# invesalius/invesalius3

Measured on AMD Instinct MI355X. Metric: Mvoxel/s segmentation + Mtriangles/s marching-cubes, 512^3 int16, 1/2/4/8 GPU, higher is better.
Workload: dtype i16; 1 GPU; configs[1]: 512x512x512 int16 per GPU, threshold(226..3071) + 26-neighbour region-grow + marching-cubes(mask@127); global_voxels=134217728, parallelism=z-slab x1, collectives=none, overlap=none

## Files before the change

### invesalius3_amd/csrc/k_flood.hip

```cpp
#include <math.h>
#include <map>
#include <mutex>
#include <stdlib.h>

#include "flood_tiles.h"

typedef short short8_t __attribute__((ext_vector_type(8)));

namespace {

constexpr int NT = TY * TZ;
constexpr int HY = TY + 2, HZ = TZ + 2;
constexpr int BATCH = 8;
constexpr int SUB = 1;
constexpr unsigned int CLOSED = 0x40u;

template <typename T> __device__ __forceinline__ double as_double(T v) { return (double)v; }

template <typename T, int BAR>
__global__ __launch_bounds__(256) void k_flood_candidates16(const short8_t *__restrict__ data,
                                                            const uint4 *__restrict__ bar, int64_t nchunks, double t0,
                                                            double t1, double fill, uint16_t *__restrict__ cand) {
    const int64_t stride = (int64_t)gridDim.x * blockDim.x;
    const int lo = (int)ceil(t0 < -70000.0 ? -70000.0 : t0), hi = (int)floor(t1 > 70000.0 ? 70000.0 : t1);
    const unsigned fb = (unsigned)(uint8_t)fill;
    for (int64_t c = (int64_t)blockIdx.x * blockDim.x + threadIdx.x; c < nchunks; c += stride) {
        const short8_t a = __builtin_nontemporal_load(&data[2 * c]);
        const short8_t b = __builtin_nontemporal_load(&data[2 * c + 1]);
        uint4 q = make_uint4(0, 0, 0, 0);
        if (BAR == 1) q = bar[c];
        const unsigned bw[4] = {q.x, q.y, q.z, q.w};
        unsigned m = 0;
#pragma unroll
        for (int e = 0; e < 16; e++) {
            const int v = (int)(T)(e < 8 ? a[e & 7] : b[e & 7]);
            bool ok = v >= lo && v <= hi;
            if (BAR == 1) ok = ok && ((bw[e >> 2] >> (8 * (e & 3))) & 0xffu) != fb;
            if (BAR == 2) ok = ok && (double)v != fill;
            m |= ok ? (1u << e) : 0u;
        }
        cand[c] = (uint16_t)m;
    }
}

template <int BAR>
__global__ __launch_bounds__(256) void k_flood_candidates16_ranges(const short8_t *__restrict__ data,
                                                                   const uint4 *__restrict__ bar,
                                                                   const unsigned *__restrict__ ranges, int64_t nchunks,
                                                                   double t0, double t1, double fill,
                                                                   uint16_t *__restrict__ cand) {
    const int64_t stride = (int64_t)gridDim.x * blockDim.x;
    const int lo = (int)ceil(t0 < -70000.0 ? -70000.0 : t0), hi = (int)floor(t1 > 70000.0 ? 70000.0 : t1);
    const unsigned fb = (unsigned)(uint8_t)fill;
    int64_t c = (int64_t)blockIdx.x * blockDim.x + threadIdx.x;
    if (c >= nchunks) return;
    unsigned rec = ranges[c >> 2];
    for (;;) {
        const int64_t cn = c + stride;
        unsigned rec_next = 0;
        if (cn < nchunks) rec_next = ranges[cn >> 2];
        const int mn = (int)(short)(rec & 0xffffu), mx = (int)(short)(rec >> 16);
        unsigned m = 0;
        if (!(mx < lo || mn > hi)) {
            const bool inside = mn >= lo && mx <= hi;
            if (inside) {
                m = 0xffffu;
            } else {
                const short8_t a = __builtin_nontemporal_load(&data[2 * c]);
                const short8_t b = __builtin_nontemporal_load(&data[2 * c + 1]);
#pragma unroll
                for (int e = 0; e < 16; e++) {
                    const int v = (int)(e < 8 ? a[e & 7] : b[e & 7]);
                    m |= (v >= lo && v <= hi) ? (1u << e) : 0u;
                }
            }
            if (BAR == 1 && m) {
                const uint4 q = bar[c];
                const unsigned bw[4] = {q.x, q.y, q.z, q.w};
#pragma unroll
                for (int e = 0; e < 16; e++)
                    if (((bw[e >> 2] >> (8 * (e & 3))) & 0xffu) == fb) m &= ~(1u << e);
            }
        }
        cand[c] = (uint16_t)m;
        if (cn >= nchunks) break;
        c = cn;
        rec = rec_next;
    }
}

template <typename T, int BAR>
__global__ __launch_bounds__(256) void k_flood_candidates(const T *__restrict__ data, const uint8_t *__restrict__ bar,
                                                          Tiles t, double t0, double t1, double fill,
                                                          uint8_t *__restrict__ cand) {
    const int64_t bpr = t.wx * 8;
    const int64_t total = t.dz * t.dy * bpr;
    const int64_t stride = (int64_t)gridDim.x * blockDim.x;
    const bool vec = (sizeof(T) == 2) && (t.dx % 8 == 0) && (((uintptr_t)data & 15) == 0) &&
                     (BAR != 1 || ((uintptr_t)bar & 7) == 0);
    for (int64_t i = (int64_t)blockIdx.x * blockDim.x + threadIdx.x; i < total; i += stride) {
        const int64_t row = i / bpr, q = i - row * bpr;
        const int64_t x0 = q * 8;
        unsigned m = 0;
        if (x0 < t.dx) {
            const int64_t base = row * t.dx + x0;
            if (vec) {
                const short8_t v = *reinterpret_cast<const short8_t *>(data + base);
                unsigned long long b8 = 0;
                if (BAR == 1) b8 = *reinterpret_cast<const unsigned long long *>(bar + base);
#pragma unroll
                for (int e = 0; e < 8; e++) {
                    const double d = (double)(T)v[e];
                    bool ok = d >= t0 && d <= t1;
                    if (BAR == 1) ok = ok && (((b8 >> (8 * e)) & 0xff) != (unsigned long long)(uint8_t)fill);
                    if (BAR == 2) ok = ok && d != fill;
                    m |= ok ? (1u << e) : 0u;
                }
            } else {
#pragma unroll
                for (int e = 0; e < 8; e++) {
                    if (x0 + e < t.dx) {
                        const double d = as_double(data[base + e]);
                        bool ok = d >= t0 && d <= t1;
                        if (BAR == 1) ok = ok && bar[base + e] != (uint8_t)fill;
                        if (BAR == 2) ok = ok && d != fill;
                        m |= ok ? (1u << e) : 0u;
                    }
                }
            }
        }
        cand[i] = (uint8_t)m;
    }
}

template <typename T>
__global__ void k_flood_seed(const T *__restrict__ data, Tiles t, double t0, double t1, const int64_t *__restrict__ seeds,
                             int64_t nseeds, unsigned long long *__restrict__ cand,
                             unsigned long long *__restrict__ reached, uint8_t *__restrict__ dirty) {
    const int64_t n = (int64_t)blockIdx.x * blockDim.x + threadIdx.x;
    if (n >= nseeds) return;
    const int64_t x = seeds[3 * n], y = seeds[3 * n + 1], z = seeds[3 * n + 2];
    const double v = as_double(data[(z * t.dy + y) * t.dx + x]);
    if (!(v >= t0 && v <= t1)) return;
    const int64_t w = (z * t.dy + y) * t.wx + (x >> 6);
    const unsigned long long bit = 1ull << (x & 63);
    atomicOr(&cand[w], bit);
    atomicOr(&reached[w], bit);
    mark_tile_nbhd(t, dirty, z / TZ, y / TY, x >> 6);
}

struct SeedPack {
    int64_t xyz[16][3];
    int n;
};
template <typename T>
__global__ void k_flood_seed_args(const T *__restrict__ data, Tiles t, double t0, double t1, SeedPack sp,
                                  unsigned long long *__restrict__ cand, unsigned long long *__restrict__ reached,
                                  uint8_t *__restrict__ dirty) {
    const int n = threadIdx.x;
    if (n >= sp.n) return;
    const int64_t x = sp.xyz[n][0], y = sp.xyz[n][1], z = sp.xyz[n][2];
    const double v = as_double(data[(z * t.dy + y) * t.dx + x]);
    if (!(v >= t0 && v <= t1)) return;
    const int64_t w = (z * t.dy + y) * t.wx + (x >> 6);
    const unsigned long long bit = 1ull << (x & 63);
    atomicOr(&cand[w], bit);
    atomicOr(&reached[w], bit);
    mark_tile_nbhd(t, dirty, z / TZ, y / TY, x >> 6);
}

__device__ __forceinline__ unsigned long long fill_up(unsigned long long seed, unsigned long long m) {
    return (((m + seed) ^ m) & m) | seed;
}
__device__ __forceinline__ unsigned long long fill_runs(unsigned long long seed, unsigned long long m) {
    unsigned long long f = fill_up(seed, m);
    return __brevll(fill_up(__brevll(f), __brevll(m)));
}

__device__ __forceinline__ void lds_barrier() {
    __builtin_amdgcn_s_waitcnt(0xC07F);
    __builtin_amdgcn_s_barrier();
}
struct TileOpen {
    unsigned long long sO[HZ * HY];
};
struct TileLds {
    unsigned long long sN[HZ * HY];
    unsigned long long sD[HZ * HY];
    unsigned char sCL[HZ * HY], sCR[HZ * HY];
    unsigned int dirs;
    unsigned int open;
    unsigned int vote[2];
};
__device__ __forceinline__ void post_dirs(TileLds &L, unsigned dirs) {
#pragma unroll
    for (int o = 32; o > 0; o >>= 1) dirs |= __shfl_xor(dirs, o, 64);
    if ((threadIdx.x & 63) == 0 && dirs) atomicOr(&L.dirs, dirs);
}

template <int CONN>
__device__ __forceinline__ void tile_update(const Tiles &t, const unsigned long long *__restrict__ cand,
                                            unsigned long long *reached, int64_t tile, TileLds &L, TileOpen &O) {
    const int64_t txi = tile % t.wx, r1 = tile / t.wx;
    const int64_t tyi = r1 % t.nty, tzi = r1 / t.nty;
    const int64_t z0 = tzi * TZ, y0 = tyi * TY;
    unsigned long long w3[2][3] = {{0ull, 0ull, 0ull}, {0ull, 0ull, 0ull}};
    unsigned long long hc[2] = {0ull, 0ull};
    unsigned int hx[2] = {0u, 0u};
#pragma unroll
    for (int pass = 0; pass < 2; pass++) {
        const int idx = threadIdx.x + pass * NT;
        if (idx < HZ * HY) {
            const int yy = idx % HY, zz = idx / HY;
            const int64_t z = z0 + zz - 1, y = y0 + yy - 1;
            if (z >= 0 && z < t.dz && y >= 0 && y < t.dy) {
                unsigned long long *row = reached + (z * t.dy + y) * t.wx;
#pragma unroll
                for (int xx = 0; xx < 3; xx++) {
                    const int64_t w = txi + xx - 1;
                    if (w >= 0 && w < t.wx) w3[pass][xx] = row[w];
                }
                if (zz == 0 || zz == HZ - 1 || yy == 0 || yy == HY - 1) hc[pass] = cand[(z * t.dy + y) * t.wx + txi];
                hx[pass] = 1u;
            }
        }
    }
#pragma unroll
    for (int pass = 0; pass < 2; pass++) {
        const int idx = threadIdx.x + pass * NT;
// ... 767 lines not shown
            auto bytes = [](unsigned int bits4) { return ((bits4 * 0x00204081u) & 0x01010101u) * 0xffu; };
            auto word = [&](unsigned int r4, unsigned int i4) {
                const unsigned int rs = bytes(r4);
                return (sel4 & rs) | (in4 & bytes(i4) & ~rs);
            };
            out[i0 + u * 256] = make_uint4(word(m[u] & 15u, b[u] & 15u), word(m[u] >> 4 & 15u, b[u] >> 4 & 15u),
                                           word(m[u] >> 8 & 15u, b[u] >> 8 & 15u), word(m[u] >> 12 & 15u, b[u] >> 12 & 15u));
        }
    }
}

__global__ __launch_bounds__(256) void k_flood_apply2(Tiles t, const uint8_t *__restrict__ reached, uint8_t *__restrict__ out,
                                                      uint8_t fill, uint8_t *__restrict__ mask, uint8_t select) {
    const int64_t bpr = t.wx * 8;
    const int64_t total = t.dz * t.dy * bpr;
    const int64_t stride = (int64_t)gridDim.x * blockDim.x;
    const bool aligned8 = (((uintptr_t)out | (uintptr_t)mask) & 7) == 0;
    for (int64_t i = (int64_t)blockIdx.x * blockDim.x + threadIdx.x; i < total; i += stride) {
        const unsigned m = reached[i];
        if (!m) continue;
        const int64_t row = i / bpr, q = i - row * bpr;
        const int64_t base = row * t.dx + q * 8;
        if (m == 0xffu && ((t.dx & 7) == 0) && aligned8) {
            *reinterpret_cast<unsigned long long *>(out + base) = 0x0101010101010101ull * fill;
            *reinterpret_cast<unsigned long long *>(mask + base) = 0x0101010101010101ull * select;
            continue;
        }
#pragma unroll
        for (int e = 0; e < 8; e++)
            if (m >> e & 1u) {
                out[base + e] = fill;
                mask[base + e] = select;
            }
    }
}

__global__ __launch_bounds__(256) void k_flood_count(const unsigned long long *__restrict__ bits, int64_t nwords,
                                                     unsigned long long *__restrict__ total) {
    unsigned long long s = 0;
    const int64_t stride = (int64_t)gridDim.x * blockDim.x;
    for (int64_t i = (int64_t)blockIdx.x * blockDim.x + threadIdx.x; i < nwords; i += stride) s += __popcll(bits[i]);
#pragma unroll
    for (int o = 32; o > 0; o >>= 1) s += __shfl_xor(s, o, 64);
    if ((threadIdx.x & 63) == 0 && s) atomicAdd(total, s);
}

static inline int grid_for(int64_t n) {
    const int64_t b = ivx::cdiv(n, 256);
    return (int)(b < 1 ? 1 : (b < 32768 ? b : 32768));
}

template <typename T>
static int run_candidates(const Tiles &t, const void *data, double t0, double t1, const uint8_t *bar, int bar_mode,
                          double fill, uint8_t *cand, hipStream_t st) {
    const int64_t total = t.dz * t.dy * t.wx * 8;
    if (!total) return IVX_OK;
    if (sizeof(T) == 2 && t.dx % 64 == 0 && (((uintptr_t)data | (uintptr_t)bar | (uintptr_t)cand) & 15) == 0) {
        const int64_t nchunks = t.dz * t.dy * t.dx / 16;
        const int64_t blocks = ivx::cdiv(nchunks, 256);
        const int gg = (int)(blocks < 16384 ? blocks : 16384);
        const short8_t *d8 = (const short8_t *)data;
        const uint4 *b4 = (const uint4 *)bar;
        uint16_t *c16 = (uint16_t *)cand;
        if (bar_mode == 0) hipLaunchKernelGGL((k_flood_candidates16<T, 0>), dim3(gg), dim3(256), 0, st, d8, b4, nchunks, t0, t1, fill, c16);
        else if (bar_mode == 1) hipLaunchKernelGGL((k_flood_candidates16<T, 1>), dim3(gg), dim3(256), 0, st, d8, b4, nchunks, t0, t1, fill, c16);
        else hipLaunchKernelGGL((k_flood_candidates16<T, 2>), dim3(gg), dim3(256), 0, st, d8, b4, nchunks, t0, t1, fill, c16);
        IVX_LAUNCH_CHECK();
        return IVX_OK;
    }
    const int g = grid_for(total);
    if (bar_mode == 0)
        hipLaunchKernelGGL((k_flood_candidates<T, 0>), dim3(g), dim3(256), 0, st, (const T *)data, bar, t, t0, t1, fill, cand);
    else if (bar_mode == 1)
        hipLaunchKernelGGL((k_flood_candidates<T, 1>), dim3(g), dim3(256), 0, st, (const T *)data, bar, t, t0, t1, fill, cand);
    else
        hipLaunchKernelGGL((k_flood_candidates<T, 2>), dim3(g), dim3(256), 0, st, (const T *)data, bar, t, t0, t1, fill, cand);
    IVX_LAUNCH_CHECK();
    return IVX_OK;
}

}

extern "C" int ivx_flood_bits_bytes(const ivx_flood_plan *p, size_t *nbytes) {
    Tiles t;
    int rc = make_tiles(p, &t);
    if (rc) return rc;
    *nbytes = al256((size_t)(t.dz * t.dy * t.wx) * 8);
    return IVX_OK;
}

extern "C" int ivx_flood_scratch_bytes(const ivx_flood_plan *p, size_t *nbytes) {
    Tiles t;
    int rc = make_tiles(p, &t);
    if (rc) return rc;
    *nbytes = make_fscratch(t).total;
    return IVX_OK;
}

extern "C" int ivx_flood_strct_bits(const uint8_t *strct, const int64_t sshape[3], uint32_t *bits) {
    IVX_REQUIRE(strct && sshape, IVX_EINVAL, "flood: strct is NULL");
    uint32_t b = 0;
    for (int a = 0; a < 3; a++)
        IVX_REQUIRE(sshape[a] >= 1 && sshape[a] <= 3, IVX_EINVAL, "flood: structuring element dims must be 1..3 (got %lld)",
                    (long long)sshape[a]);
    const int64_t oz = sshape[0] / 2, oy = sshape[1] / 2, ox = sshape[2] / 2;
    for (int64_t kk = 0; kk < sshape[0]; kk++)
        for (int64_t jj = 0; jj < sshape[1]; jj++)
            for (int64_t ii = 0; ii < sshape[2]; ii++)
                if (strct[(kk * sshape[1] + jj) * sshape[2] + ii]) {
                    const int64_t dz = kk - oz + 1, dy = jj - oy + 1, dx = ii - ox + 1;
                    b |= 1u << (dz * 9 + dy * 3 + dx);
                }
    *bits = b;
    return IVX_OK;
}

extern "C" int ivx_dev_flood_candidates(const ivx_flood_plan *p, int dtype, const void *data, double t0, double t1,
                                        const uint8_t *barrier, int barrier_mode, double fill, uint64_t *cand,
                                        void *stream) {
    Tiles t;
    int rc = make_tiles(p, &t);
    if (rc) return rc;
    IVX_REQUIRE(barrier_mode >= 0 && barrier_mode <= 2, IVX_EINVAL, "flood: barrier_mode");
    IVX_REQUIRE(barrier_mode != 1 || barrier, IVX_EINVAL, "flood: barrier array missing");
    hipStream_t st = ivx::S(stream);
    switch (dtype) {
    case IVX_I16: return run_candidates<int16_t>(t, data, t0, t1, barrier, barrier_mode, fill, (uint8_t *)cand, st);
    case IVX_U8: return run_candidates<uint8_t>(t, data, t0, t1, barrier, barrier_mode, fill, (uint8_t *)cand, st);
    case IVX_U16: return run_candidates<uint16_t>(t, data, t0, t1, barrier, barrier_mode, fill, (uint8_t *)cand, st);
    case IVX_F64: return run_candidates<double>(t, data, t0, t1, barrier, barrier_mode, fill, (uint8_t *)cand, st);
    }
    ivx::set_error("flood: unsupported dtype %d", dtype);
    return IVX_EINVAL;
}

extern "C" int ivx_dev_flood_candidates_ranges(const ivx_flood_plan *p, const int16_t *data, double t0, double t1,
                                               const uint8_t *barrier, int barrier_mode, double fill,
                                               const uint32_t *ranges, uint64_t *cand, void *stream) {
    Tiles t;
    int rc = make_tiles(p, &t);
    if (rc) return rc;
    IVX_REQUIRE(barrier_mode == 0 || barrier_mode == 1, IVX_EINVAL, "flood: candidates_ranges: barrier_mode 0 or 1");
    IVX_REQUIRE(barrier_mode != 1 || barrier, IVX_EINVAL, "flood: barrier array missing");
    IVX_REQUIRE(t.dx % 64 == 0 && (((uintptr_t)data | (uintptr_t)barrier | (uintptr_t)cand) & 15) == 0 && ((uintptr_t)ranges & 3) == 0,
                IVX_EINVAL, "flood: candidates_ranges needs dx %% 64 == 0, 16-byte aligned buffers and 4-byte aligned records "
                            "(use ivx_dev_flood_candidates)");
    const int64_t nchunks = t.dz * t.dy * t.dx / 16;
    if (!nchunks) return IVX_OK;
    IVX_REQUIRE(data && ranges && cand, IVX_EINVAL, "flood: candidates_ranges: null argument");
    const int64_t blocks = ivx::cdiv(nchunks, 256);
    const int gg = (int)(blocks < 16384 ? blocks : 16384);
    hipStream_t st = ivx::S(stream);
    if (barrier_mode == 0)
        hipLaunchKernelGGL((k_flood_candidates16_ranges<0>), dim3(gg), dim3(256), 0, st, (const short8_t *)data, (const uint4 *)barrier,
                           (const unsigned *)ranges, nchunks, t0, t1, fill, (uint16_t *)cand);
    else
        hipLaunchKernelGGL((k_flood_candidates16_ranges<1>), dim3(gg), dim3(256), 0, st, (const short8_t *)data, (const uint4 *)barrier,
                           (const unsigned *)ranges, nchunks, t0, t1, fill, (uint16_t *)cand);
    IVX_LAUNCH_CHECK();
    return IVX_OK;
}

extern "C" int ivx_dev_flood_seed(const ivx_flood_plan *p, int dtype, const void *data, double t0, double t1,
                                  const int64_t *seeds_xyz, int64_t nseeds, uint64_t *cand, uint64_t *reached,
                                  void *scratch_, void *stream) {
    Tiles t;
    int rc = make_tiles(p, &t);
    if (rc) return rc;
    for (int64_t n = 0; n < nseeds; n++) {
        const int64_t x = seeds_xyz[3 * n], y = seeds_xyz[3 * n + 1], z = seeds_xyz[3 * n + 2];
        IVX_REQUIRE(x >= 0 && y >= 0 && z >= 0 && x < t.dx && y < t.dy && z < t.dz, IVX_ERANGE,
                    "flood: seed (%lld,%lld,%lld) outside volume (%lld,%lld,%lld) [x,y,z]", (long long)x, (long long)y,
                    (long long)z, (long long)t.dx, (long long)t.dy, (long long)t.dz);
    }
    const FScratch s = make_fscratch(t);
    char *scr = (char *)scratch_;
    hipStream_t st = ivx::S(stream);
    ivx::ccl_invalidate(scratch_);
    if (nseeds <= 16) {
        SeedPack sp;
        sp.n = (int)nseeds;
        for (int64_t n = 0; n < nseeds; n++)
            for (int q = 0; q < 3; q++) sp.xyz[n][q] = seeds_xyz[3 * n + q];
        unsigned long long *c = (unsigned long long *)cand, *r = (unsigned long long *)reached;
        uint8_t *dirty = (uint8_t *)(scr + s.off_dirty0);
        if (nseeds == 0) return IVX_OK;
        switch (dtype) {
        case IVX_I16: hipLaunchKernelGGL(k_flood_seed_args<int16_t>, dim3(1), dim3(64), 0, st, (const int16_t *)data, t, t0, t1, sp, c, r, dirty); break;
        case IVX_U8: hipLaunchKernelGGL(k_flood_seed_args<uint8_t>, dim3(1), dim3(64), 0, st, (const uint8_t *)data, t, t0, t1, sp, c, r, dirty); break;
        case IVX_U16: hipLaunchKernelGGL(k_flood_seed_args<uint16_t>, dim3(1), dim3(64), 0, st, (const uint16_t *)data, t, t0, t1, sp, c, r, dirty); break;
        case IVX_F64: hipLaunchKernelGGL(k_flood_seed_args<double>, dim3(1), dim3(64), 0, st, (const double *)data, t, t0, t1, sp, c, r, dirty); break;
        default: ivx::set_error("flood: unsupported dtype %d", dtype); return IVX_EINVAL;
        }
        IVX_LAUNCH_CHECK();
        return IVX_OK;
    }
    int64_t *d_seeds = (int64_t *)(scr + s.off_seeds);
    for (int64_t b = 0; b < nseeds; b += (int64_t)SEED_CHUNK) {
        const int64_t m = nseeds - b < (int64_t)SEED_CHUNK ? nseeds - b : (int64_t)SEED_CHUNK;
        IVX_HIP(hipMemcpyAsync(d_seeds, seeds_xyz + 3 * b, (size_t)m * 24, hipMemcpyHostToDevice, st));
        const int g = (int)ivx::cdiv(m, 256);
        unsigned long long *c = (unsigned long long *)cand, *r = (unsigned long long *)reached;
        uint8_t *dirty = (uint8_t *)(scr + s.off_dirty0);
        switch (dtype) {
        case IVX_I16: hipLaunchKernelGGL(k_flood_seed<int16_t>, dim3(g), dim3(256), 0, st, (const int16_t *)data, t, t0, t1, d_seeds, m, c, r, dirty); break;
        case IVX_U8: hipLaunchKernelGGL(k_flood_seed<uint8_t>, dim3(g), dim3(256), 0, st, (const uint8_t *)data, t, t0, t1, d_seeds, m, c, r, dirty); break;
        case IVX_U16: hipLaunchKernelGGL(k_flood_seed<uint16_t>, dim3(g), dim3(256), 0, st, (const uint16_t *)data, t, t0, t1, d_seeds, m, c, r, dirty); break;
        case IVX_F64: hipLaunchKernelGGL(k_flood_seed<double>, dim3(g), dim3(256), 0, st, (const double *)data, t, t0, t1, d_seeds, m, c, r, dirty); break;
        default: ivx::set_error("flood: unsupported dtype %d", dtype); return IVX_EINVAL;
        }
        IVX_LAUNCH_CHECK();
        IVX_HIP(hipStreamSynchronize(st));
    }
    return IVX_OK;
}

__global__ __launch_bounds__(256) void k_flood_clear(uint4 *__restrict__ reached, int64_t n16, uint4 *__restrict__ head,
                                                     int64_t h16) {
    const int64_t stride = (int64_t)gridDim.x * blockDim.x;
    const uint4 z = make_uint4(0u, 0u, 0u, 0u);
    for (int64_t i = (int64_t)blockIdx.x * blockDim.x + threadIdx.x; i < n16 + h16; i += stride) {
        if (i < n16) reached[i] = z;
        else head[i - n16] = z;
    }
}

extern "C" int ivx_dev_flood_clear(const ivx_flood_plan *p, uint64_t *reached, void *scratch, void *stream) {
    Tiles t;
    int rc = make_tiles(p, &t);
    if (rc) return rc;
    const FScratch s = make_fscratch(t);
    const size_t nb = (size_t)(t.dz * t.dy * t.wx) * 8;
    if ((nb | s.off_seeds | (uintptr_t)reached | (uintptr_t)scratch) & 15) {
        IVX_HIP(hipMemsetAsync(reached, 0, nb, ivx::S(stream)));
        IVX_HIP(hipMemsetAsync(scratch, 0, s.off_seeds, ivx::S(stream)));
    } else {
        const int64_t total = (int64_t)((nb + s.off_seeds) / 16);
        const int64_t blocks = ivx::cdiv(total, 256);
        hipLaunchKernelGGL(k_flood_clear, dim3((unsigned)(blocks < 8192 ? blocks : 8192)), dim3(256), 0, ivx::S(stream),
                           (uint4 *)reached, (int64_t)(nb / 16), (uint4 *)scratch, (int64_t)(s.off_seeds / 16));
        IVX_LAUNCH_CHECK();
    }
    ivx::ccl_invalidate(scratch);
    return IVX_OK;
}

struct GateArm {
    unsigned int *word;
    unsigned int value, below;
};
static std::map<const void *, GateArm> g_gates;
static std::mutex g_gates_mu;

__global__ void k_gate_wait(const unsigned int *word, unsigned int value, unsigned long long timeout_ticks) {
    if (threadIdx.x) return;
    const unsigned long long t0 = wall_clock64();
    while (__hip_atomic_load(word, __ATOMIC_RELAXED, __HIP_MEMORY_SCOPE_AGENT) != value) {
        if (wall_clock64() - t0 > timeout_ticks) break;
        __builtin_amdgcn_s_sleep(32);
    }
}
__global__ void k_gate_set(unsigned int *word, unsigned int value) {
    if (threadIdx.x == 0) __hip_atomic_store(word, value, __ATOMIC_RELAXED, __HIP_MEMORY_SCOPE_AGENT);
}

struct Fresh {
    int dtype;
    const void *data;
    double t0, t1;
    SeedPack sp;
};
static bool flood_mode_ccl() {
    static const bool ccl = [] {
        const char *e = getenv("IVX_FLOOD_MODE");
        return e && !strcmp(e, "ccl");
    }();
    return ccl;
}
static bool coarse_ok(const Tiles &t, ivx::FloodMode mode) {
    static const bool coarse_on = [] {
        const char *e = getenv("IVX_FLOOD_COARSE");
        return !(e && e[0] == '0');
    }();
    return coarse_on && mode == ivx::FLOOD_SYMMETRIC && t.conn != 0 && t.wx <= 64 && (t.nty + 2) * (t.ntz + 2) <= CROWS_MAX &&
           t.nty * t.ntz <= (int64_t)CT * CRP;
}
static Blocks coarse_blocks(const Tiles &t) {
    static const int bxs_env = [] {
        const char *e = getenv("IVX_FLOOD_BLOCK");
        return e ? atoi(e) : 0;
    }();
    Blocks bk;
    bk.bxs = 16;
    while (bk.bxs < 64 && ((64 / bk.bxs) * t.wx > 64 || bk.bxs < bxs_env)) bk.bxs *= 2;
    bk.q = 64 / bk.bxs;
    return bk;
}
static int coarse_lanes(const Tiles &t) {
    int ct = 64;
    while (ct < CT && ct < t.nty * t.ntz) ct *= 2;
    return ct;
}
template <bool FRESH>
static int coarse_pass(const Tiles &t, const FScratch &s, char *scr, const uint64_t *cand, uint64_t *reached, const Fresh &f,
                       int ncnt, hipStream_t st) {
    const Blocks bk = coarse_blocks(t);
    uint8_t *dirty0 = (uint8_t *)(scr + s.off_dirty0), *dirty1 = (uint8_t *)(scr + s.off_dirty1);
    unsigned int *cnt = (unsigned int *)(scr + s.off_cnt), *list0 = (unsigned int *)(scr + s.off_list0);
    unsigned long long *rowF = (unsigned long long *)(scr + s.off_full), *rowW = (unsigned long long *)(scr + s.off_whole);
    unsigned int *seed_ok = (unsigned int *)(scr + s.off_status) + 8;
// ... 687 lines not shown
```

### invesalius3_amd/csrc/k_threshold.hip

```cpp
#include "ivx_internal.h"

typedef short short8_t __attribute__((ext_vector_type(8)));
typedef unsigned char uchar16_t __attribute__((ext_vector_type(16)));

namespace {

__device__ __forceinline__ unsigned char keep_or(unsigned char m, unsigned char v) {
    return (m == 1 || m == 2 || m == 253 || m == 254) ? m : v;
}

template <bool PRESERVE>
__global__ __launch_bounds__(256) void k_threshold16(const short8_t *__restrict__ img, uchar16_t *__restrict__ mask,
                                                     int64_t nchunks, int lo, int hi,
                                                     const uint8_t *__restrict__ skip, int64_t chunks_per_slice) {
    const int64_t stride = (int64_t)gridDim.x * blockDim.x;
    for (int64_t c = (int64_t)blockIdx.x * blockDim.x + threadIdx.x; c < nchunks; c += stride) {
        if (skip && skip[c / chunks_per_slice]) continue;
        const short8_t a = __builtin_nontemporal_load(&img[2 * c]);
        const short8_t b = __builtin_nontemporal_load(&img[2 * c + 1]);
        uchar16_t r;
#pragma unroll
        for (int i = 0; i < 8; i++) {
            r[i] = ((int)a[i] >= lo && (int)a[i] <= hi) ? 255 : 0;
            r[8 + i] = ((int)b[i] >= lo && (int)b[i] <= hi) ? 255 : 0;
        }
        if (PRESERVE) {
            const uchar16_t m = mask[c];
#pragma unroll
            for (int i = 0; i < 16; i++) r[i] = keep_or(m[i], r[i]);
        }
        mask[c] = r;
    }
}

__global__ __launch_bounds__(256) void k_threshold16_bits(const short8_t *__restrict__ img, uchar16_t *__restrict__ mask,
                                                          uint16_t *__restrict__ bits, int64_t nchunks, int lo, int hi) {
    const int64_t stride = (int64_t)gridDim.x * blockDim.x;
    for (int64_t c = (int64_t)blockIdx.x * blockDim.x + threadIdx.x; c < nchunks; c += stride) {
        const short8_t a = __builtin_nontemporal_load(&img[2 * c]);
        const short8_t b = __builtin_nontemporal_load(&img[2 * c + 1]);
        uchar16_t r;
        unsigned m = 0;
#pragma unroll
        for (int i = 0; i < 8; i++) {
            const bool in0 = (int)a[i] >= lo && (int)a[i] <= hi, in1 = (int)b[i] >= lo && (int)b[i] <= hi;
            r[i] = in0 ? 255 : 0;
            r[8 + i] = in1 ? 255 : 0;
            m |= (in0 ? 1u : 0u) << i;
            m |= (in1 ? 1u : 0u) << (8 + i);
        }
        mask[c] = r;
        bits[c] = (uint16_t)m;
    }
}

__device__ __forceinline__ int quad_xor1(int v) { return __builtin_amdgcn_update_dpp(v, v, 0xB1, 0xf, 0xf, true); }
__device__ __forceinline__ int quad_xor2(int v) { return __builtin_amdgcn_update_dpp(v, v, 0x4E, 0xf, 0xf, true); }

__device__ __forceinline__ unsigned word_record(const short8_t a, const short8_t b) {
    int mn = a[0], mx = a[0];
#pragma unroll
    for (int i = 0; i < 8; i++) {
        mn = min(mn, min((int)a[i], (int)b[i]));
        mx = max(mx, max((int)a[i], (int)b[i]));
    }
    mn = min(mn, quad_xor1(mn));
    mx = max(mx, quad_xor1(mx));
    mn = min(mn, quad_xor2(mn));
    mx = max(mx, quad_xor2(mx));
    return ((unsigned)mn & 0xffffu) | ((unsigned)mx << 16);
}

__global__ __launch_bounds__(256) void k_image_ranges16(const short8_t *__restrict__ img, unsigned *__restrict__ ranges,
                                                        int64_t nchunks) {
    const int64_t stride = (int64_t)gridDim.x * blockDim.x;
    for (int64_t c = (int64_t)blockIdx.x * blockDim.x + threadIdx.x; c < nchunks; c += stride) {
        const short8_t a = __builtin_nontemporal_load(&img[2 * c]);
        const short8_t b = __builtin_nontemporal_load(&img[2 * c + 1]);
        const unsigned rec = word_record(a, b);
        if ((c & 3) == 0) ranges[c >> 2] = rec;
    }
}

__global__ __launch_bounds__(256) void k_threshold16_bits_build(const short8_t *__restrict__ img, uchar16_t *__restrict__ mask,
                                                                uint16_t *__restrict__ bits, unsigned *__restrict__ ranges,
                                                                int64_t nchunks, int lo, int hi) {
    const int64_t stride = (int64_t)gridDim.x * blockDim.x;
    for (int64_t c = (int64_t)blockIdx.x * blockDim.x + threadIdx.x; c < nchunks; c += stride) {
        const short8_t a = __builtin_nontemporal_load(&img[2 * c]);
        const short8_t b = __builtin_nontemporal_load(&img[2 * c + 1]);
        uchar16_t r;
        unsigned m = 0;
#pragma unroll
        for (int i = 0; i < 8; i++) {
            const bool in0 = (int)a[i] >= lo && (int)a[i] <= hi, in1 = (int)b[i] >= lo && (int)b[i] <= hi;
            r[i] = in0 ? 255 : 0;
            r[8 + i] = in1 ? 255 : 0;
            m |= (in0 ? 1u : 0u) << i;
            m |= (in1 ? 1u : 0u) << (8 + i);
        }
        const unsigned rec = word_record(a, b);
        mask[c] = r;
        bits[c] = (uint16_t)m;
        if ((c & 3) == 0) ranges[c >> 2] = rec;
    }
}

__global__ __launch_bounds__(256) void k_threshold16_bits_use(const short8_t *__restrict__ img, uchar16_t *__restrict__ mask,
                                                              uint16_t *__restrict__ bits, const unsigned *__restrict__ ranges,
                                                              int64_t nchunks, int lo, int hi) {
    const int64_t stride = (int64_t)gridDim.x * blockDim.x;
    int64_t c = (int64_t)blockIdx.x * blockDim.x + threadIdx.x;
    if (c >= nchunks) return;
    unsigned rec = ranges[c >> 2];
    for (;;) {
        const int64_t cn = c + stride;
        unsigned rec_next = 0;
        if (cn < nchunks) rec_next = ranges[cn >> 2];
        const int mn = (int)(short)(rec & 0xffffu), mx = (int)(short)(rec >> 16);
        uchar16_t r;
        unsigned m;
        if (mn >= lo && mx <= hi) {
#pragma unroll
            for (int i = 0; i < 16; i++) r[i] = 255;
            m = 0xffffu;
        } else if (mx < lo || mn > hi) {
#pragma unroll
            for (int i = 0; i < 16; i++) r[i] = 0;
            m = 0;
        } else {
            const short8_t a = __builtin_nontemporal_load(&img[2 * c]);
            const short8_t b = __builtin_nontemporal_load(&img[2 * c + 1]);
            m = 0;
#pragma unroll
            for (int i = 0; i < 8; i++) {
                const bool in0 = (int)a[i] >= lo && (int)a[i] <= hi, in1 = (int)b[i] >= lo && (int)b[i] <= hi;
                r[i] = in0 ? 255 : 0;
                r[8 + i] = in1 ? 255 : 0;
                m |= (in0 ? 1u : 0u) << i;
                m |= (in1 ? 1u : 0u) << (8 + i);
            }
        }
        mask[c] = r;
        bits[c] = (uint16_t)m;
        if (cn >= nchunks) break;
        c = cn;
        rec = rec_next;
    }
}

__device__ __forceinline__ unsigned chunk_bits(const short8_t a, const short8_t b, int lo, int hi) {
    unsigned m = 0;
#pragma unroll
    for (int i = 0; i < 8; i++) {
        const bool in0 = (int)a[i] >= lo && (int)a[i] <= hi, in1 = (int)b[i] >= lo && (int)b[i] <= hi;
        m |= (in0 ? 1u : 0u) << i;
        m |= (in1 ? 1u : 0u) << (8 + i);
    }
    return m;
}

template <bool BUILD>
__global__ __launch_bounds__(256) void k_threshold16_plane(const short8_t *__restrict__ img, uint16_t *__restrict__ bits,
                                                           unsigned *__restrict__ ranges, int64_t nchunks, int lo, int hi) {
    const int64_t stride = (int64_t)gridDim.x * blockDim.x;
    for (int64_t c = (int64_t)blockIdx.x * blockDim.x + threadIdx.x; c < nchunks; c += stride) {
        const short8_t a = __builtin_nontemporal_load(&img[2 * c]);
        const short8_t b = __builtin_nontemporal_load(&img[2 * c + 1]);
        bits[c] = (uint16_t)chunk_bits(a, b, lo, hi);
        if (BUILD) {
            const unsigned rec = word_record(a, b);
            if ((c & 3) == 0) ranges[c >> 2] = rec;
        }
    }
}

__global__ __launch_bounds__(256) void k_threshold16_plane_use(const short8_t *__restrict__ img, uint16_t *__restrict__ bits,
                                                               const unsigned *__restrict__ ranges, int64_t nchunks, int lo,
                                                               int hi) {
    const int64_t stride = (int64_t)gridDim.x * blockDim.x;
    int64_t c = (int64_t)blockIdx.x * blockDim.x + threadIdx.x;
    if (c >= nchunks) return;
    unsigned rec = ranges[c >> 2];
    for (;;) {
        const int64_t cn = c + stride;
        unsigned rec_next = 0;
        if (cn < nchunks) rec_next = ranges[cn >> 2];
        const int mn = (int)(short)(rec & 0xffffu), mx = (int)(short)(rec >> 16);
        unsigned m;
        if (mn >= lo && mx <= hi) {
            m = 0xffffu;
        } else if (mx < lo || mn > hi) {
            m = 0;
        } else {
            const short8_t a = __builtin_nontemporal_load(&img[2 * c]);
            const short8_t b = __builtin_nontemporal_load(&img[2 * c + 1]);
            m = chunk_bits(a, b, lo, hi);
        }
        bits[c] = (uint16_t)m;
        if (cn >= nchunks) break;
        c = cn;
        rec = rec_next;
    }
}

template <bool PRESERVE>
__global__ __launch_bounds__(256) void k_threshold1(const int16_t *__restrict__ img, uint8_t *__restrict__ mask,
                                                    int64_t begin, int64_t n, int lo, int hi,
                                                    const uint8_t *__restrict__ skip, int64_t slice_elems) {
    const int64_t stride = (int64_t)gridDim.x * blockDim.x;
    for (int64_t i = begin + (int64_t)blockIdx.x * blockDim.x + threadIdx.x; i < n; i += stride) {
        if (skip && skip[i / slice_elems]) continue;
        const int v = img[i];
        unsigned char r = (v >= lo && v <= hi) ? 255 : 0;
        if (PRESERVE) r = keep_or(mask[i], r);
        mask[i] = r;
    }
}

}

extern "C" int ivx_dev_threshold_i16(const int16_t *img, int64_t dz, int64_t dy, int64_t dx, int lo, int hi,
                                     int preserve, const uint8_t *skip_flags, uint8_t *mask, void *stream) {
    IVX_REQUIRE(dz >= 0 && dy >= 0 && dx >= 0, IVX_EINVAL, "threshold: negative shape");
    const int64_t slice = dy * dx, n = dz * slice;
    if (n == 0) return IVX_OK;
    const bool aligned = (((uintptr_t)img | (uintptr_t)mask) & 15) == 0;
    const bool vec_ok = aligned && (!skip_flags || slice % 16 == 0);
    int64_t done = 0;
    if (vec_ok && n >= 16) {
        const int64_t nchunks = n / 16;
        const int64_t blocks = ivx::cdiv(nchunks, 256);
        const int grid = (int)(blocks < 16384 ? blocks : 16384);
        const int64_t cps = skip_flags ? slice / 16 : 1;
        if (preserve)
            hipLaunchKernelGGL(k_threshold16<true>, dim3(grid), dim3(256), 0, ivx::S(stream), (const short8_t *)img,
                               (uchar16_t *)mask, nchunks, lo, hi, skip_flags, cps);
        else
            hipLaunchKernelGGL(k_threshold16<false>, dim3(grid), dim3(256), 0, ivx::S(stream), (const short8_t *)img,
                               (uchar16_t *)mask, nchunks, lo, hi, skip_flags, cps);
        IVX_LAUNCH_CHECK();
        done = nchunks * 16;
    }
    if (done < n) {
        const int64_t rem = n - done;
        const int64_t blocks = ivx::cdiv(rem, 256);
        const int grid = (int)(blocks < 16384 ? blocks : 16384);
        if (preserve)
            hipLaunchKernelGGL(k_threshold1<true>, dim3(grid), dim3(256), 0, ivx::S(stream), img, mask, done, n, lo, hi,
                               skip_flags, slice);
        else
            hipLaunchKernelGGL(k_threshold1<false>, dim3(grid), dim3(256), 0, ivx::S(stream), img, mask, done, n, lo,
                               hi, skip_flags, slice);
        IVX_LAUNCH_CHECK();
    }
    return IVX_OK;
}

extern "C" int ivx_dev_threshold_i16_bits(const int16_t *img, int64_t dz, int64_t dy, int64_t dx, int lo, int hi,
                                          uint8_t *mask, uint64_t *bits, void *stream) {
    IVX_REQUIRE(dz >= 0 && dy >= 0 && dx >= 0, IVX_EINVAL, "threshold: negative shape");
    IVX_REQUIRE(dx % 64 == 0 && (((uintptr_t)img | (uintptr_t)mask | (uintptr_t)bits) & 15) == 0, IVX_EINVAL,
                "threshold_bits: needs dx %% 64 == 0 and 16-byte aligned buffers (use ivx_dev_threshold_i16)");
    const int64_t n = dz * dy * dx;
    if (n == 0) return IVX_OK;
    const int64_t nchunks = n / 16;
    const int64_t blocks = ivx::cdiv(nchunks, 256);
    hipLaunchKernelGGL(k_threshold16_bits, dim3((unsigned)(blocks < 16384 ? blocks : 16384)), dim3(256), 0, ivx::S(stream),
                       (const short8_t *)img, (uchar16_t *)mask, (uint16_t *)bits, nchunks, lo, hi);
    IVX_LAUNCH_CHECK();
    return IVX_OK;
}

extern "C" int ivx_image_ranges_bytes(int64_t dz, int64_t dy, int64_t dx, size_t *nbytes) {
    IVX_REQUIRE(nbytes, IVX_EINVAL, "image_ranges: nbytes is NULL");
    IVX_REQUIRE(dz >= 0 && dy >= 0 && dx >= 0, IVX_EINVAL, "image_ranges: negative shape");
    IVX_REQUIRE(dx % 64 == 0, IVX_EINVAL, "image_ranges: needs dx %% 64 == 0 (rows of whole 64-voxel words)");
    *nbytes = (size_t)(dz * dy * (dx / 64)) * 4;
    return IVX_OK;
}

static inline unsigned ranges_grid(int64_t nchunks) {
    const int64_t blocks = ivx::cdiv(nchunks, 256);
    return (unsigned)(blocks < 16384 ? blocks : 16384);
}

extern "C" int ivx_dev_image_ranges_i16(const int16_t *img, int64_t dz, int64_t dy, int64_t dx, uint32_t *ranges,
                                        void *stream) {
    IVX_REQUIRE(dz >= 0 && dy >= 0 && dx >= 0, IVX_EINVAL, "image_ranges: negative shape");
    IVX_REQUIRE(dx % 64 == 0 && ((uintptr_t)img & 15) == 0 && ((uintptr_t)ranges & 3) == 0, IVX_EINVAL,
                "image_ranges: needs dx %% 64 == 0, a 16-byte aligned image and 4-byte aligned records");
    const int64_t n = dz * dy * dx;
    if (n == 0) return IVX_OK;
    IVX_REQUIRE(img && ranges, IVX_EINVAL, "image_ranges: null argument");
    hipLaunchKernelGGL(k_image_ranges16, dim3(ranges_grid(n / 16)), dim3(256), 0, ivx::S(stream), (const short8_t *)img,
                       (unsigned *)ranges, n / 16);
    IVX_LAUNCH_CHECK();
    return IVX_OK;
}

extern "C" int ivx_dev_threshold_i16_bits_ranges(const int16_t *img, int64_t dz, int64_t dy, int64_t dx, int lo, int hi,
                                                 uint8_t *mask, uint64_t *bits, uint32_t *ranges, int mode, void *stream) {
    IVX_REQUIRE(dz >= 0 && dy >= 0 && dx >= 0, IVX_EINVAL, "threshold: negative shape");
    IVX_REQUIRE(dx % 64 == 0 && (((uintptr_t)img | (uintptr_t)mask | (uintptr_t)bits) & 15) == 0 && ((uintptr_t)ranges & 3) == 0,
                IVX_EINVAL, "threshold_bits_ranges: needs dx %% 64 == 0, 16-byte aligned buffers and 4-byte aligned records "
                            "(use ivx_dev_threshold_i16)");
    IVX_REQUIRE(mode == IVX_RANGES_BUILD || mode == IVX_RANGES_USE, IVX_EINVAL, "threshold_bits_ranges: mode %d", mode);
    const int64_t n = dz * dy * dx;
    if (n == 0) return IVX_OK;
    IVX_REQUIRE(img && mask && bits && ranges, IVX_EINVAL, "threshold_bits_ranges: null argument");
    const int64_t nchunks = n / 16;
    if (mode == IVX_RANGES_BUILD)
        hipLaunchKernelGGL(k_threshold16_bits_build, dim3(ranges_grid(nchunks)), dim3(256), 0, ivx::S(stream),
                           (const short8_t *)img, (uchar16_t *)mask, (uint16_t *)bits, (unsigned *)ranges, nchunks, lo, hi);
    else
        hipLaunchKernelGGL(k_threshold16_bits_use, dim3(ranges_grid(nchunks)), dim3(256), 0, ivx::S(stream),
                           (const short8_t *)img, (uchar16_t *)mask, (uint16_t *)bits, (const unsigned *)ranges, nchunks, lo, hi);
    IVX_LAUNCH_CHECK();
    return IVX_OK;
}

extern "C" int ivx_dev_threshold_i16_plane(const int16_t *img, int64_t dz, int64_t dy, int64_t dx, int lo, int hi, uint64_t *bits,
                                           void *stream) {
    IVX_REQUIRE(dz >= 0 && dy >= 0 && dx >= 0, IVX_EINVAL, "threshold: negative shape");
    IVX_REQUIRE(dx % 64 == 0 && (((uintptr_t)img | (uintptr_t)bits) & 15) == 0, IVX_EINVAL,
                "threshold_plane: needs dx %% 64 == 0 and 16-byte aligned buffers");
    const int64_t n = dz * dy * dx;
    if (n == 0) return IVX_OK;
    IVX_REQUIRE(img && bits, IVX_EINVAL, "threshold_plane: null argument");
    const int64_t nchunks = n / 16;
    hipLaunchKernelGGL(k_threshold16_plane<false>, dim3(ranges_grid(nchunks)), dim3(256), 0, ivx::S(stream), (const short8_t *)img,
                       (uint16_t *)bits, (unsigned *)nullptr, nchunks, lo, hi);
    IVX_LAUNCH_CHECK();
    return IVX_OK;
}

extern "C" int ivx_dev_threshold_i16_plane_ranges(const int16_t *img, int64_t dz, int64_t dy, int64_t dx, int lo, int hi,
                                                  uint64_t *bits, uint32_t *ranges, int mode, void *stream) {
    IVX_REQUIRE(dz >= 0 && dy >= 0 && dx >= 0, IVX_EINVAL, "threshold: negative shape");
    IVX_REQUIRE(dx % 64 == 0 && (((uintptr_t)img | (uintptr_t)bits) & 15) == 0 && ((uintptr_t)ranges & 3) == 0, IVX_EINVAL,
                "threshold_plane_ranges: needs dx %% 64 == 0, 16-byte aligned buffers and 4-byte aligned records");
    IVX_REQUIRE(mode == IVX_RANGES_BUILD || mode == IVX_RANGES_USE, IVX_EINVAL, "threshold_plane_ranges: mode %d", mode);
    const int64_t n = dz * dy * dx;
    if (n == 0) return IVX_OK;
    IVX_REQUIRE(img && bits && ranges, IVX_EINVAL, "threshold_plane_ranges: null argument");
    const int64_t nchunks = n / 16;
    if (mode == IVX_RANGES_BUILD)
        hipLaunchKernelGGL(k_threshold16_plane<true>, dim3(ranges_grid(nchunks)), dim3(256), 0, ivx::S(stream),
                           (const short8_t *)img, (uint16_t *)bits, (unsigned *)ranges, nchunks, lo, hi);
    else
        hipLaunchKernelGGL(k_threshold16_plane_use, dim3(ranges_grid(nchunks)), dim3(256), 0, ivx::S(stream),
                           (const short8_t *)img, (uint16_t *)bits, (const unsigned *)ranges, nchunks, lo, hi);
    IVX_LAUNCH_CHECK();
    return IVX_OK;
}

extern "C" int ivx_threshold_all_slices(const int16_t *img, const int64_t shape[3], const int64_t ist[3], int lo,
                                        int hi, int preserve, int honour_flags, uint8_t *mask,
                                        const int64_t mst[3]) {
    ivx::HostCallGuard host_guard__;
    using namespace ivx;
    const int64_t dz = shape[0], dy = shape[1], dx = shape[2];
    IVX_REQUIRE(dz >= 0 && dy >= 0 && dx >= 0, IVX_EINVAL, "threshold: negative shape");
    const size_t n = (size_t)dz * dy * dx;
    if (n == 0) return IVX_OK;
    void *d_img, *d_mask, *d_flags;
    int rc;
    if ((rc = ws_get(WS_IN, n * 2, &d_img))) return rc;
    if ((rc = ws_get(WS_OUT, n, &d_mask))) return rc;
    if ((rc = ws_get(WS_SMALL, (size_t)dz, &d_flags))) return rc;
    if ((rc = upload_strided(d_img, img, shape, ist, 2, WS_IN))) return rc;
    uint8_t *inner = mask + mst[0] + mst[1] + mst[2];
    bool any_skip = false;
    void *hflags;
    if ((rc = hs_get(WS_SMALL, (size_t)dz, &hflags))) return rc;
    uint8_t *hf = (uint8_t *)hflags;
    for (int64_t z = 0; z < dz; z++) {
        hf[z] = honour_flags ? mask[(z + 1) * mst[0]] : 0;
        any_skip |= hf[z] != 0;
    }
    if (preserve || any_skip) {
        if ((rc = upload_strided(d_mask, inner, shape, mst, 1, WS_OUT))) return rc;
    }
    if (any_skip) IVX_HIP(hipMemcpy(d_flags, hf, (size_t)dz, hipMemcpyHostToDevice));
    rc = ivx_dev_threshold_i16((const int16_t *)d_img, dz, dy, dx, lo, hi, preserve,
                               any_skip ? (const uint8_t *)d_flags : nullptr, (uint8_t *)d_mask, nullptr);
    if (rc) return rc;
    IVX_HIP(hipDeviceSynchronize());
    if ((rc = download_strided(inner, shape, mst, d_mask, 1, WS_OUT))) return rc;
    for (int64_t z = 0; z < dz; z++) mask[(z + 1) * mst[0]] = honour_flags && hf[z] ? hf[z] : 1;
    const int64_t fshape[3] = {1, 1, dz}, fst[3] = {0, 0, mst[0]};
    return mirror_host_view(mask + mst[0], fshape, fst, 1, d_flags, WS_SMALL);
}
```

Baseline: 404,100 Mvoxel/s.

## Compact mixed 64-voxel words across lanes when building bit-planes from range records

Replaces the per-16-voxel chunk loop in the threshold and no-barrier flood-candidate kernels with a shared word-level routine. Each lane owns one 64-voxel word. Only words whose min/max record straddles the threshold are compacted with ballot and permute, so the whole wavefront cooperatively loads and tests just those words and reassembles 64-bit masks through DPP and bpermute. This targets divergence and wasted lanes when few words are mixed, and replaces 16-bit stores with 64-bit ones. The cost is more cross-lane shuffle work, and the code now assumes one range record per 64-voxel word.

```diff
diff --git a/invesalius3_amd/csrc/k_flood.hip b/invesalius3_amd/csrc/k_flood.hip
--- a/invesalius3_amd/csrc/k_flood.hip
+++ b/invesalius3_amd/csrc/k_flood.hip
@@ -4,8 +4,7 @@
 #include <stdlib.h>
 
 #include "flood_tiles.h"
-
-typedef short short8_t __attribute__((ext_vector_type(8)));
+#include "words_from_records.h"
 
 namespace {
 
@@ -43,7 +42,13 @@
     }
 }
 
-template <int BAR>
+__global__ __launch_bounds__(256) void k_flood_candidates_words(const short8_t *__restrict__ data, const unsigned *__restrict__ ranges,
+                                                                int64_t nwords, double t0, double t1,
+                                                                unsigned long long *__restrict__ cand) {
+    const int lo = (int)ceil(t0 < -70000.0 ? -70000.0 : t0), hi = (int)floor(t1 > 70000.0 ? 70000.0 : t1);
+    words_from_records(data, ranges, nwords, lo, hi, cand);
+}
+
 __global__ __launch_bounds__(256) void k_flood_candidates16_ranges(const short8_t *__restrict__ data,
                                                                    const uint4 *__restrict__ bar,
                                                                    const unsigned *__restrict__ ranges, int64_t nchunks,
@@ -74,7 +79,7 @@
                     m |= (v >= lo && v <= hi) ? (1u << e) : 0u;
                 }
             }
-            if (BAR == 1 && m) {
+            if (m) {
                 const uint4 q = bar[c];
                 const unsigned bw[4] = {q.x, q.y, q.z, q.w};
 #pragma unroll
@@ -1148,10 +1153,10 @@
     const int gg = (int)(blocks < 16384 ? blocks : 16384);
     hipStream_t st = ivx::S(stream);
     if (barrier_mode == 0)
-        hipLaunchKernelGGL((k_flood_candidates16_ranges<0>), dim3(gg), dim3(256), 0, st, (const short8_t *)data, (const uint4 *)barrier,
-                           (const unsigned *)ranges, nchunks, t0, t1, fill, (uint16_t *)cand);
+        hipLaunchKernelGGL(k_flood_candidates_words, dim3(words_grid(nchunks / 4)), dim3(WORDS_PER_WG), 0, st, (const short8_t *)data,
+                           (const unsigned *)ranges, nchunks / 4, t0, t1, (unsigned long long *)cand);
     else
-        hipLaunchKernelGGL((k_flood_candidates16_ranges<1>), dim3(gg), dim3(256), 0, st, (const short8_t *)data, (const uint4 *)barrier,
+        hipLaunchKernelGGL(k_flood_candidates16_ranges, dim3(gg), dim3(256), 0, st, (const short8_t *)data, (const uint4 *)barrier,
                            (const unsigned *)ranges, nchunks, t0, t1, fill, (uint16_t *)cand);
     IVX_LAUNCH_CHECK();
     return IVX_OK;
diff --git a/invesalius3_amd/csrc/k_threshold.hip b/invesalius3_amd/csrc/k_threshold.hip
--- a/invesalius3_amd/csrc/k_threshold.hip
+++ b/invesalius3_amd/csrc/k_threshold.hip
@@ -1,6 +1,6 @@
 #include "ivx_internal.h"
-
-typedef short short8_t __attribute__((ext_vector_type(8)));
+#include "words_from_records.h"
+
 typedef unsigned char uchar16_t __attribute__((ext_vector_type(16)));
 
 namespace {
@@ -53,9 +53,6 @@
         bits[c] = (uint16_t)m;
     }
 }
-
-__device__ __forceinline__ int quad_xor1(int v) { return __builtin_amdgcn_update_dpp(v, v, 0xB1, 0xf, 0xf, true); }
-__device__ __forceinline__ int quad_xor2(int v) { return __builtin_amdgcn_update_dpp(v, v, 0x4E, 0xf, 0xf, true); }
 
 __device__ __forceinline__ unsigned word_record(const short8_t a, const short8_t b) {
     int mn = a[0], mx = a[0];
@@ -175,33 +172,10 @@
     }
 }
 
-__global__ __launch_bounds__(256) void k_threshold16_plane_use(const short8_t *__restrict__ img, uint16_t *__restrict__ bits,
-                                                               const unsigned *__restrict__ ranges, int64_t nchunks, int lo,
+__global__ __launch_bounds__(256) void k_threshold16_plane_use(const short8_t *__restrict__ img, unsigned long long *__restrict__ bits,
+                                                               const unsigned *__restrict__ ranges, int64_t nwords, int lo,
                                                                int hi) {
-    const int64_t stride = (int64_t)gridDim.x * blockDim.x;
-    int64_t c = (int64_t)blockIdx.x * blockDim.x + threadIdx.x;
-    if (c >= nchunks) return;
-    unsigned rec = ranges[c >> 2];
-    for (;;) {
-        const int64_t cn = c + stride;
-        unsigned rec_next = 0;
-        if (cn < nchunks) rec_next = ranges[cn >> 2];
-        const int mn = (int)(short)(rec & 0xffffu), mx = (int)(short)(rec >> 16);
-        unsigned m;
-        if (mn >= lo && mx <= hi) {
-            m = 0xffffu;
-        } else if (mx < lo || mn > hi) {
-            m = 0;
-        } else {
-            const short8_t a = __builtin_nontemporal_load(&img[2 * c]);
-            const short8_t b = __builtin_nontemporal_load(&img[2 * c + 1]);
-            m = chunk_bits(a, b, lo, hi);
-        }
-        bits[c] = (uint16_t)m;
-        if (cn >= nchunks) break;
-        c = cn;
-        rec = rec_next;
-    }
+    words_from_records(img, ranges, nwords, lo, hi, bits);
 }
 
 template <bool PRESERVE>
@@ -349,8 +323,8 @@
         hipLaunchKernelGGL(k_threshold16_plane<true>, dim3(ranges_grid(nchunks)), dim3(256), 0, ivx::S(stream),
                            (const short8_t *)img, (uint16_t *)bits, (unsigned *)ranges, nchunks, lo, hi);
     else
-        hipLaunchKernelGGL(k_threshold16_plane_use, dim3(ranges_grid(nchunks)), dim3(256), 0, ivx::S(stream),
-                           (const short8_t *)img, (uint16_t *)bits, (const unsigned *)ranges, nchunks, lo, hi);
+        hipLaunchKernelGGL(k_threshold16_plane_use, dim3(words_grid(n / 64)), dim3(WORDS_PER_WG), 0, ivx::S(stream),
+                           (const short8_t *)img, (unsigned long long *)bits, (const unsigned *)ranges, n / 64, lo, hi);
     IVX_LAUNCH_CHECK();
     return IVX_OK;
 }
diff --git a/invesalius3_amd/csrc/words_from_records.h b/invesalius3_amd/csrc/words_from_records.h
--- /dev/null
+++ b/invesalius3_amd/csrc/words_from_records.h
@@ -0,0 +1,74 @@
+#pragma once
+#include "ivx_internal.h"
+
+typedef short short8_t __attribute__((ext_vector_type(8)));
+
+namespace {
+
+__device__ __forceinline__ int quad_xor1(int v) { return __builtin_amdgcn_update_dpp(v, v, 0xB1, 0xf, 0xf, true); }
+__device__ __forceinline__ int quad_xor2(int v) { return __builtin_amdgcn_update_dpp(v, v, 0x4E, 0xf, 0xf, true); }
+__device__ __forceinline__ int half_mirror(int v) { return __builtin_amdgcn_update_dpp(v, v, 0x141, 0xf, 0xf, true); }
+
+constexpr int WORDS_PER_WG = 256;
+
+static inline unsigned words_grid(int64_t nwords) { return (unsigned)ivx::cdiv(nwords, WORDS_PER_WG); }
+
+template <int NP>
+__device__ __forceinline__ void words_mixed_passes(const short8_t *__restrict__ line0, int owner_of, int nmix, int rank, bool mixed,
+                                                   int lo, int hi, unsigned &w_lo, unsigned &w_hi) {
+    const int lane = threadIdx.x & 63, grp = lane >> 3, seg = lane & 7;
+    short8_t d[NP];
+#pragma unroll
+    for (int p = 0; p < NP; p++) {
+        const int k = min(8 * p + grp, nmix - 1);
+        const int src = __builtin_amdgcn_ds_bpermute(k << 2, owner_of);
+        d[p] = __builtin_nontemporal_load(&line0[src * 8]);
+    }
+    const int from = (rank & 7) << 5;
+#pragma unroll
+    for (int p = 0; p < NP; p++) {
+        unsigned b = 0;
+#pragma unroll
+        for (int i = 0; i < 8; i++) b |= ((int)d[p][i] >= lo && (int)d[p][i] <= hi ? 1u : 0u) << i;
+        int x = (int)(b << (8 * (seg & 3)));
+        x |= quad_xor1(x);
+        x |= quad_xor2(x);
+        const int y = half_mirror(x);
+        const int t_lo = __builtin_amdgcn_ds_bpermute(from, seg < 4 ? x : y);
+        const int t_hi = __builtin_amdgcn_ds_bpermute(from, seg < 4 ? y : x);
+        if (mixed && (rank >> 3) == p) {
+            w_lo = (unsigned)t_lo;
+            w_hi = (unsigned)t_hi;
+        }
+    }
+}
+
+__device__ __forceinline__ void words_from_records(const short8_t *__restrict__ img, const unsigned *__restrict__ ranges,
+                                                   int64_t nwords, int lo, int hi, unsigned long long *__restrict__ plane) {
+    const int lane = threadIdx.x & 63;
+    const int64_t wbase = (int64_t)blockIdx.x * WORDS_PER_WG + __builtin_amdgcn_readfirstlane((int)(threadIdx.x & 192u));
+    const int64_t w = wbase + lane;
+    const bool valid = w < nwords;
+    unsigned rec = 0;
+    if (valid) rec = ranges[w];
+    const int mn = (int)(short)(rec & 0xffffu), mx = (int)(short)(rec >> 16);
+    const bool inside = mn >= lo && mx <= hi;
+    const bool mixed = valid && !inside && !(mx < lo || mn > hi);
+    unsigned w_lo = inside ? ~0u : 0u, w_hi = w_lo;
+    const unsigned long long mk = __ballot(mixed);
+    if (mk) {
+        const int nmix = __popcll(mk);
+        const int rank = (int)__builtin_amdgcn_mbcnt_hi((unsigned)(mk >> 32), __builtin_amdgcn_mbcnt_lo((unsigned)mk, 0u));
+        const int owner_of = __builtin_amdgcn_ds_permute((mixed ? rank : nmix + lane - rank) << 2, lane);
+        const short8_t *line0 = img + wbase * 8 + (lane & 7);
+        if (nmix <= 8) words_mixed_passes<1>(line0, owner_of, nmix, rank, mixed, lo, hi, w_lo, w_hi);
+        else if (nmix <= 16) words_mixed_passes<2>(line0, owner_of, nmix, rank, mixed, lo, hi, w_lo, w_hi);
+        else if (nmix <= 24) words_mixed_passes<3>(line0, owner_of, nmix, rank, mixed, lo, hi, w_lo, w_hi);
+        else if (nmix <= 32) words_mixed_passes<4>(line0, owner_of, nmix, rank, mixed, lo, hi, w_lo, w_hi);
+        else if (nmix <= 48) words_mixed_passes<6>(line0, owner_of, nmix, rank, mixed, lo, hi, w_lo, w_hi);
+        else words_mixed_passes<8>(line0, owner_of, nmix, rank, mixed, lo, hi, w_lo, w_hi);
+    }
+    if (valid) plane[w] = ((unsigned long long)w_hi << 32) | w_lo;
+}
+
+}
```

Result: faster. 424,600 Mvoxel/s (median of 6 runs) (+5.1%).
